# orottier/web-audio-api-rs

Measured on AMD Instinct MI355X. Metric: render quanta/sec (48kHz, 128-frame), higher is better.
Workload: dtype f64

## Files before the change

### web-audio-api-rs_amd/csrc/waa_internal.hpp

```cpp
#pragma once
#include <cstdint>
#include <cstdlib>

#include "waa_conv_noise.hpp"

namespace waa {

inline const char* measure_switch(const char* name) {
#ifdef WAA_MEASURE
  return getenv(name);
#else
  (void)name;
  return nullptr;
#endif
}

void raise_lds_limit(const void* kernel);

constexpr int RQ = 128;
constexpr int TILE_K = 32;
constexpr int TILE = 64 * TILE_K;
constexpr int QUANTA_PER_TILE = TILE / RQ;
constexpr int MAX_OPS = 12;
constexpr int MAX_INPUTS = 4;
constexpr int MAX_CH = 32;
constexpr int STATE_STRIDE = MAX_CH * 4;

struct ParamRef {
  const float* base;
  uint64_t stride;
  int32_t mode;
  int32_t pad;
};

struct SignalRef {
  float* base;
  uint64_t inst_stride;
  uint64_t ch_stride;
  int32_t nch;
  int32_t pad;
};

enum : uint32_t { Q_SILENT = 0, Q_FAST = 1, Q_SLOW = 2, Q_FAST_LOOP = 3 };
struct QRec {
  int64_t start;
  uint32_t mode;
  uint32_t pad;
};
struct SlowRec {
  int32_t prev;
  int32_t next;
  double k;
};
struct SrcSchedule {
  const QRec* qrec;
  const SlowRec* slow;
  const uint8_t* tile_fast;
};
struct SrcInst {
  const float* base;
// ... 304 lines not shown
  int32_t type;
  const uint32_t* wave_row;
  SignalRef out;
  uint64_t frames;
  uint32_t n_inst;
  uint32_t n_quanta;
  double sample_rate;
  const struct OscQuantum* table_q;
  const uint32_t* tq_row;
  const int64_t* active;
  const double* start_ratio;
  double* seg_phase;
  ParamRef post_gain[2];
  int32_t n_post;
  int32_t post_dup;
  const struct OscQuantum* fm_q;
  const uint32_t* fm_row;
  const float* fm_table;
  const uint32_t* fm_wave_row;
  int32_t fm_table_len, fm_type;
  ParamRef fm_gain;
  int32_t fm_has_gain;
  float fm_min, fm_max, fm_default;
  int32_t pa_on;
  float pa_min, pa_max, pa_default;
  ParamRef pa_intrinsic;
};
constexpr int OSC_SEGMENTS = 8;
struct OscQuantum {
  double phase;
  double incr;
  int16_t first, end;
  int32_t outside_nyquist;
};
void launch_osc(const OscDesc& d, void* stream);

constexpr int PERIODIC_WAVE_LEN = 8192;
struct PeriodicWaveDesc {
  const float* real;
  const float* imag;
  const uint32_t* normalize;
  const uint32_t* dst_row;
  float* tables;
  uint32_t n;
  uint32_t rows;
};
void launch_periodic_wave(const PeriodicWaveDesc& d, void* stream);

enum : int32_t { LI_NODE = 0, LI_DELAY_W = 1, LI_DELAY_R = 2 };
constexpr int LOOP_MAX_ITEMS = 24;
struct LoopItem {
  int32_t kind;
  int32_t nch_in;
  int32_t nch_out;
  int32_t interp;
  int32_t n_in;
  int32_t in_item[MAX_INPUTS];
  int32_t in_nch[MAX_INPUTS];
  SignalRef in_sig[MAX_INPUTS];
  SignalRef out;
  OpDesc op;
  int32_t writer_item;
  int32_t in_cycle;
  int32_t num_quanta;
  int32_t pad;
};
// ... 373 lines not shown
```

### web-audio-api-rs_amd/csrc/waa_kernels.hip

```cpp
#include <hip/hip_runtime.h>

#include <cstdlib>

#include "waa_curve.hpp"
#include "waa_internal.hpp"
#include "waa_mix.hpp"

namespace waa {

constexpr int LDS_ROW = TILE_K + 4;
constexpr int CARRY_BYTES = MAX_OPS * 8 * 4 * 8;

struct f4 {
  float x, y, z, w;
};

__device__ __forceinline__ float param_at(const ParamRef& p, uint32_t inst, uint32_t q, uint64_t frame) {
  if (p.mode == 0) return p.base[inst];
  if (p.mode == 1) return p.base[(uint64_t)inst * p.stride + q];
  return p.base[(uint64_t)inst * p.stride + frame];
}


template <int C, int K>
__device__ __forceinline__ void load_input(const InputRef& in, uint32_t inst, uint32_t tile, int lane, uint32_t n_quanta,
                                           float (&v)[C][K]) {
  constexpr int NV4 = K / 4;
  constexpr int TILE_FR = 64 * K;
  constexpr int QPT = K / 2;
  const uint64_t f_tile = (uint64_t)tile * TILE_FR;
  if (in.kind == IN_SIGNAL) {
#pragma unroll
    for (int c = 0; c < C; c++) {
      if (c < in.nch) {
        const float* p = in.sig.base + (uint64_t)inst * in.sig.inst_stride + (uint64_t)c * in.sig.ch_stride + f_tile;
#pragma unroll
        for (int j = 0; j < NV4; j++) {
          const bool inside = in.valid == 0 || f_tile + (uint64_t)(j * 256 + lane * 4) + 3 < in.valid;
// ... 191 lines not shown
__device__ __forceinline__ void gain_regs(float (&v)[C][K], int nch, const ParamRef& p0, uint32_t inst, uint32_t tile, int lane,
                                          uint32_t n_quanta) {
  constexpr int NV4 = K / 4;
  constexpr int TILE_FR = 64 * K;
  constexpr int QPT = K / 2;
#pragma unroll
  for (int j = 0; j < NV4; j++) {
    const uint32_t q = tile * QPT + j * 2 + (lane >> 5);
    const uint32_t qc = q < n_quanta ? q : n_quanta - 1;
    const uint64_t f = (uint64_t)tile * TILE_FR + j * 256 + lane * 4;
    if (p0.mode == 2) {
#pragma unroll
      for (int e = 0; e < 4; e++) {
        const uint64_t fc = f + e < (uint64_t)n_quanta * RQ ? f + e : (uint64_t)n_quanta * RQ - 1;
        const float g = p0.base[(uint64_t)inst * p0.stride + fc];
#pragma unroll
        for (int c = 0; c < C; c++)
          if (c < nch) v[c][j * 4 + e] *= g;
      }
    } else {
      const float g = param_at(p0, inst, qc, 0);
      const bool mute = fabsf(g) <= 1e-6f;
      const bool pass = fabsf(1.f - g) <= 1e-6f;
#pragma unroll
      for (int c = 0; c < C; c++)
        if (c < nch) {
#pragma unroll
          for (int e = 0; e < 4; e++) v[c][j * 4 + e] = mute ? 0.f : (pass ? v[c][j * 4 + e] : v[c][j * 4 + e] * g);
        }
    }
  }
}

struct Mat2 {
  double a, b, c, d;
};
__device__ __forceinline__ Mat2 matmul(const Mat2& x, const Mat2& y) {
  Mat2 r;
  r.a = __builtin_fma(x.a, y.a, x.b * y.c);
  r.b = __builtin_fma(x.a, y.b, x.b * y.d);
  r.c = __builtin_fma(x.c, y.a, x.d * y.c);
  r.d = __builtin_fma(x.c, y.b, x.d * y.d);
  return r;
}
__device__ __forceinline__ double shfl_up_d(double v, int delta) { return __shfl_up(v, delta, 64); }

template <int C>
__device__ __forceinline__ void biquad_op(const OpDesc& op, uint32_t inst, uint32_t tile, int lane, uint32_t n_quanta,
                                          float* lds, float (&v)[C][TILE_K], double* carry, const double* coef_inst) {
  constexpr int NV4 = TILE_K / 4;
  const int nch = op.nch_in;
#pragma unroll
  for (int c = 0; c < C; c++) {
    if (c < nch) {
      float* base = lds + c * (64 * LDS_ROW);
#pragma unroll
      for (int j = 0; j < NV4; j++) {
        const int row = j * 8 + (lane >> 3), col = (lane & 7) * 4;
        *reinterpret_cast<float4*>(base + row * LDS_ROW + col) =
            make_float4(v[c][j * 4 + 0], v[c][j * 4 + 1], v[c][j * 4 + 2], v[c][j * 4 + 3]);
      }
    }
  }
  __syncthreads();
  const bool per_frame = op.i0 == 2;
  const uint64_t f_lane = (uint64_t)tile * TILE + (uint64_t)lane * TILE_K;
// ... 121 lines not shown
            make_float4(yo[j * 4 + 0], yo[j * 4 + 1], yo[j * 4 + 2], yo[j * 4 + 3]);
    }
  }
  __syncthreads();
#pragma unroll
  for (int c = 0; c < C; c++) {
    if (c < nch) {
      const float* base = lds + c * (64 * LDS_ROW);
#pragma unroll
      for (int j = 0; j < NV4; j++) {
        const int row = j * 8 + (lane >> 3), col = (lane & 7) * 4;
        const float4 t = *reinterpret_cast<const float4*>(base + row * LDS_ROW + col);
        v[c][j * 4 + 0] = t.x;
        v[c][j * 4 + 1] = t.y;
        v[c][j * 4 + 2] = t.z;
        v[c][j * 4 + 3] = t.w;
      }
    }
  }
  __syncthreads();
}


__device__ __forceinline__ void stereo_gains_dev(float x, float& gl, float& gr) {
  const float PI_F = 3.14159265358979323846f;
  gl = sinf((1.f - x) * PI_F / 2.f);
  gr = sinf(x * PI_F / 2.f);
}

template <int C, int K, bool SERIAL, bool FANIN = true, bool PERSIST = false, bool NOSPILL = false>
__global__ __launch_bounds__(SERIAL ? 64 : 256)
    __attribute__((amdgpu_waves_per_eu((!SERIAL && FANIN && C == 2) ? (NOSPILL ? 5 : 6) : 1)))
void chain_kernel(const ChainDesc d) {
  extern __shared__ __attribute__((aligned(16))) float lds[];
  constexpr int NV4 = K / 4;
  constexpr int TILE_FR = 64 * K;
  constexpr int QPT = K / 2;
  const int lane = threadIdx.x & 63;
  const uint32_t n_tiles_k = (d.tile1 - d.tile0) * (TILE / TILE_FR);
  uint32_t inst, tile_first, tile_last;
  uint32_t tile_step = 1, per_block = 0;
  if (SERIAL) {
    inst = blockIdx.x;
    tile_first = d.tile0 * (TILE / TILE_FR);
    tile_last = d.tile1 * (TILE / TILE_FR);
  } else if (PERSIST) {
    inst = blockIdx.x;
    tile_first = d.tile0 * (TILE / TILE_FR) + (uint32_t)__builtin_amdgcn_readfirstlane((int)(threadIdx.x >> 6));
    tile_last = d.tile1 * (TILE / TILE_FR);
    tile_step = 4;
    per_block = d.persist_block / 4;
  } else {
    uint32_t blk = blockIdx.x;
    if (d.xcd_remap) {
      const uint32_t q = gridDim.x / 8, r = gridDim.x % 8, x = blk % 8, j = blk / 8;
      blk = x * q + (x < r ? x : r) + j;
    }
    const uint64_t wid = (uint64_t)blk * 4 + (uint32_t)__builtin_amdgcn_readfirstlane((int)(threadIdx.x >> 6));
    if (d.tile_major) {
      inst = (uint32_t)(wid % d.n_inst);
      tile_first = d.tile0 * (TILE / TILE_FR) + (uint32_t)(wid / d.n_inst);
      if (wid / d.n_inst >= n_tiles_k) inst = d.n_inst;
    } else {
      inst = (uint32_t)(wid / n_tiles_k);
      tile_first = d.tile0 * (TILE / TILE_FR) + (uint32_t)(wid % n_tiles_k);
    }
// ... 3 lines not shown
    if (d.lds_curve_op >= 0) {
      const int nn = d.ops[d.lds_curve_op].i0;
      const float* src = reinterpret_cast<const float*>(d.ops[d.lds_curve_op].ptr0);
      for (int i = threadIdx.x; i < nn; i += 256) lds[i] = src[i];
      __syncthreads();
    }
  }
  if (inst >= d.n_inst) return;
  __builtin_amdgcn_s_setreg(1 | (6 << 6) | (1 << 11), 0);

  double* carry_all = reinterpret_cast<double*>(lds + C * 64 * LDS_ROW);
  if constexpr (SERIAL) {
    for (int o = 0; o < d.n_ops; o++) {
      if (d.ops[o].kind == OP_BIQUAD) {
        const double* st = reinterpret_cast<const double*>(d.ops[o].ptr1) + (uint64_t)inst * STATE_STRIDE;
        if (lane < C * 4) carry_all[o * C * 4 + lane] = (lane >> 2) < d.ops[o].nch_in ? st[lane] : 0.;
      }
    }
    __syncthreads();
  }

  uint32_t done_in_block = 0;
  for (uint32_t tile = tile_first; tile < tile_last; tile += (PERSIST ? tile_step : 1u)) {
    if constexpr (PERSIST) {
      if (per_block) {
        if (done_in_block == per_block) {
          __syncthreads();
          done_in_block = 0;
        }
        done_in_block++;
      }
    }
    float v[C][K];
    if constexpr (!FANIN) {
      load_input<C, K>(d.in[0], inst, tile, lane, d.n_quanta, v);
      if (d.in[0].has_gain) gain_regs<C, K>(v, d.in[0].nch, d.in[0].gain, inst, tile, lane, d.n_quanta);
      mix_regs<C, K>(v, d.in[0].nch, d.in_nch, d.in_interp);
    } else {
#pragma unroll
      for (int c = 0; c < C; c++) {
#pragma unroll
        for (int i = 0; i < K; i++) v[c][i] = 0.f;
      }
#pragma nounroll
      for (int k = 0; k < d.n_inputs; k++) {
        float u[C][K];
        int lane_k = lane;
        asm volatile("" : "+v"(lane_k));
        load_input<C, K>(d.in[k], inst, tile, lane_k, d.n_quanta, u);
        if (d.in[k].has_gain) gain_regs<C, K>(u, d.in[k].nch, d.in[k].gain, inst, tile, lane_k, d.n_quanta);
        mix_regs<C, K>(u, d.in[k].nch, d.in_nch, d.in_interp);
#pragma unroll
        for (int c = 0; c < C; c++)
          if (c < d.in_nch) {
#pragma unroll
            for (int i = 0; i < K; i++) v[c][i] = k == 0 ? u[c][i] : v[c][i] + u[c][i];
          }
      }
    }
    for (int o = 0; o < d.n_ops; o++) {
      const OpDesc& op = d.ops[o];
      switch (op.kind) {
        case OP_GAIN:
          gain_regs<C, K>(v, op.nch_in, op.p0, inst, tile, lane, d.n_quanta);
          break;
        case OP_PARAM_ADD: {
          const float pmin = __int_as_float(op.i0), pmax = __int_as_float(op.i1), pdef = __int_as_float(op.i2);
#pragma unroll
          for (int j = 0; j < NV4; j++) {
            const uint32_t q = tile * QPT + j * 2 + (lane >> 5);
            const uint32_t qc = q < d.n_quanta ? q : d.n_quanta - 1;
            const uint64_t f = (uint64_t)tile * TILE_FR + j * 256 + lane * 4;
#pragma unroll
            for (int e = 0; e < 4; e++) {
              const uint64_t fc = f + e < (uint64_t)d.n_quanta * RQ ? f + e : (uint64_t)d.n_quanta * RQ - 1;
              float o1 = v[0][j * 4 + e] + param_at(op.p0, inst, qc, fc);
              o1 = o1 != o1 ? pdef : fminf(fmaxf(o1, pmin), pmax);
              v[0][j * 4 + e] = o1;
            }
          }
          break;
        }
        case OP_BIQUAD: {
          if constexpr (SERIAL) {
            const double* coef = reinterpret_cast<const double*>(op.ptr0) + (uint64_t)inst * op.u0;
            biquad_op<C>(op, inst, tile, lane, d.n_quanta, lds, v, carry_all + o * C * 4, coef);
          }
          break;
        }
        case OP_WAVESHAPER: {
          if (!SERIAL && o == d.lds_curve_op) {
#pragma unroll
            for (int c = 0; c < C; c++)
              if (c < op.nch_in) {
#pragma unroll
                for (int i = 0; i < K; i++)
                  v[c][i] = apply_curve_lds((const __attribute__((address_space(3))) float*)lds, op.i0, v[c][i]);
// ... 289 lines not shown
      return;
    }
    ChainDesc dd = d;
    dd.lds_curve_op = -1;
    dd.tile_major = 0;
    for (int k = 0; k < d.n_inputs; k++) dd.tile_major |= d.in[k].kind == IN_SOURCE;
    if (measure_switch("WAA_NO_TILE_MAJOR")) dd.tile_major = 0;
    dd.xcd_remap = !dd.tile_major && !measure_switch("WAA_NO_XCD_REMAP");
    for (int o = 0; o < d.n_ops; o++)
      if (d.ops[o].kind == OP_WAVESHAPER && d.ops[o].i0 > 0 && d.ops[o].i0 <= 8192) {
        dd.lds_curve_op = o;
        break;
      }
    const size_t lds = dd.lds_curve_op >= 0 ? (size_t)d.ops[dd.lds_curve_op].i0 * sizeof(float) : 0;
    const uint64_t waves = (uint64_t)d.n_inst * (d.tile1 - d.tile0) * (TILE / 256);
    dim3 grid((unsigned)((waves + 3) / 4)), block(256);
    if (d.persist_block) {
      grid = dim3(d.n_inst);
      dd.tile_major = 0;
      dd.xcd_remap = 0;
      if (d.n_inputs <= 1) {
        if (cmax <= 1)
          hipLaunchKernelGGL((chain_kernel<1, 4, false, false, true>), grid, block, lds, s, dd);
        else
          hipLaunchKernelGGL((chain_kernel<2, 4, false, false, true>), grid, block, lds, s, dd);
      } else if (cmax <= 1) {
        hipLaunchKernelGGL((chain_kernel<1, 4, false, true, true>), grid, block, lds, s, dd);
      } else {
        hipLaunchKernelGGL((chain_kernel<2, 4, false, true, true>), grid, block, lds, s, dd);
      }
      return;
    }
    if (d.n_inputs <= 1) {
      if (cmax <= 1)
        hipLaunchKernelGGL((chain_kernel<1, 4, false, false>), grid, block, lds, s, dd);
      else if (cmax <= 2)
        hipLaunchKernelGGL((chain_kernel<2, 4, false, false>), grid, block, lds, s, dd);
      else if (cmax <= 4)
        hipLaunchKernelGGL((chain_kernel<4, 4, false, false>), grid, block, lds, s, dd);
      else
        hipLaunchKernelGGL((chain_kernel<6, 4, false, false>), grid, block, lds, s, dd);
    } else if (cmax <= 1)
      hipLaunchKernelGGL((chain_kernel<1, 4, false>), grid, block, lds, s, dd);
    else if (cmax <= 2) {
      bool frame_pan = false;
      for (int o = 0; o < d.n_ops; o++)
        frame_pan |= (d.ops[o].kind == OP_STEREO_PAN || d.ops[o].kind == OP_PANNER) && d.ops[o].p0.mode == 2;
      if (frame_pan || measure_switch("WAA_CHAIN_NOSPILL"))
        hipLaunchKernelGGL((chain_kernel<2, 4, false, true, false, true>), grid, block, lds, s, dd);
      else
        hipLaunchKernelGGL((chain_kernel<2, 4, false>), grid, block, lds, s, dd);
    } else if (cmax <= 4)
      hipLaunchKernelGGL((chain_kernel<4, 4, false>), grid, block, lds, s, dd);
    else
      hipLaunchKernelGGL((chain_kernel<6, 4, false>), grid, block, lds, s, dd);
  }
}

}
```

### web-audio-api-rs_amd/csrc/waa_osc.hip

```cpp
#include <hip/hip_runtime.h>

#include "waa_internal.hpp"

namespace waa {

namespace {
__device__ __forceinline__ double unroll_phase(double phase) {
  if (phase >= 1.) return phase - 1.;
  if (phase < 0.) return phase + 1.;
  return phase;
}
__device__ __forceinline__ double unroll_phase_unbounded(double phase) {
  const double r = fmod(phase, 1.);
  return r < 0. ? r + 1. : r;
}
__device__ __forceinline__ double poly_blep(double t, double dt) {
  if (t < dt) {
    t /= dt;
    return t + t - t * t - 1.0;
  } else if (t > 1.0 - dt) {
    t = (t - 1.0) / dt;
    return __builtin_fma(t, t, t) + t + 1.0;
  }
  return 0.0;
}
__device__ __forceinline__ float table_sample(const float* table, int len, double phase) {
  const double position = phase * (double)len;
  const double floored = floor(position);
  const int prev_index = (int)floored >= len ? 0 : (int)floored;
  int next_index = prev_index + 1;
  if (next_index == len) next_index = 0;
  const float k = (float)(position - floored);
  return __builtin_fmaf(table[prev_index], 1.f - k, table[next_index] * k);
}
__device__ __forceinline__ float waveform_sample(int type, const float* table, int table_len, double phase, double phase_incr) {
  switch (type) {
    case 1: {
      double sample = phase < 0.5 ? 1.0 : -1.0;
      sample += poly_blep(phase, phase_incr);
      sample -= poly_blep(unroll_phase(phase + 0.5), phase_incr);
      return (float)sample;
    }
    case 2: {
      const double ph = unroll_phase(phase + 0.5);
      double sample = 2.0 * ph - 1.0;
      sample -= poly_blep(ph, phase_incr);
      return (float)sample;
    }
    case 3: {
      double sample = -4. * phase + 2.;
      if (sample > 1.)
        sample = 2. - sample;
      else if (sample < -1.)
        sample = -2. - sample;
      return (float)sample;
    }
    default: return table_sample(table, table_len, phase);
  }
}
__device__ __forceinline__ const float* table_of(const float* table, const uint32_t* wave_row, int table_len, uint32_t inst) {
  return wave_row ? table + (uint64_t)wave_row[inst] * (uint64_t)table_len : table;
}
}

namespace {
__device__ __forceinline__ void osc_store(const OscDesc& d, uint32_t inst, float* out, uint64_t f0, float (&r)[4]) {
#pragma unroll
  for (int k = 0; k < 2; k++)
    if (k < d.n_post) {
      const float g = d.post_gain[k].base[inst];
      const bool mute = fabsf(g) <= 1e-6f, pass = fabsf(1.f - g) <= 1e-6f;
#pragma unroll
      for (int e = 0; e < 4; e++) r[e] = mute ? 0.f : (pass ? r[e] : r[e] * g);
    }
  if (d.pa_on) {
    const uint32_t q = (uint32_t)(f0 / RQ), qc = q < d.n_quanta ? q : d.n_quanta - 1;
    const float iv = d.pa_intrinsic.mode == 0 ? d.pa_intrinsic.base[inst] : d.pa_intrinsic.base[(uint64_t)inst * d.pa_intrinsic.stride + qc];
#pragma unroll
    for (int e = 0; e < 4; e++) {
      const float o1 = r[e] + iv;
      r[e] = o1 != o1 ? d.pa_default : fminf(fmaxf(o1, d.pa_min), d.pa_max);
    }
  }
  *reinterpret_cast<float4*>(out + f0) = make_float4(r[0], r[1], r[2], r[3]);
  if (d.post_dup) *reinterpret_cast<float4*>(out + d.out.ch_stride + f0) = make_float4(r[0], r[1], r[2], r[3]);
}
}

__global__ __launch_bounds__(64) void osc_kernel(const OscDesc d) {
  const uint32_t inst = blockIdx.x * 64 + threadIdx.x;
  if (inst >= d.n_inst) return;
  __builtin_amdgcn_s_setreg(1 | (6 << 6) | (1 << 11), 0);
  float* out = d.out.base + (uint64_t)inst * d.out.inst_stride;
  const float* table = table_of(d.table, d.wave_row, d.table_len, inst);
  double start_time = d.start[inst];
  const double stop_time = d.stop[inst];
  const double sample_rate = d.sample_rate, dt = 1. / sample_rate, nyquist = sample_rate / 2.;
  double phase = 0.;
  bool started = false;
  const bool per_frame = d.frequency.mode == 2 || d.detune.mode == 2;
  for (uint32_t q = 0; q < d.n_quanta; q++) {
    const uint64_t f0 = (uint64_t)q * RQ;
    const double block_time = (double)f0 / sample_rate;
    const double next_block_time = block_time + dt * (double)RQ;
    float4* o4 = reinterpret_cast<float4*>(out + f0);
    if (stop_time <= block_time || start_time >= next_block_time) {
      for (int j = 0; j < RQ / 4; j++) o4[j] = make_float4(0.f, 0.f, 0.f, 0.f);
      continue;
    }
    double current_time = block_time;
    if (!started && start_time < current_time) start_time = current_time;
    auto generate = [&](bool outside_nyquist, double phase_incr) __attribute__((always_inline)) -> float {
      float v = 0.f;
      if (!(current_time < start_time || current_time >= stop_time)) {
        if (!started) {
          if (current_time > start_time) {
// ... 37 lines not shown
      for (int j = 0; j < RQ / 4; j++) {
        float r[4];
#pragma unroll
        for (int e = 0; e < 4; e++) {
          const uint64_t f = f0 + j * 4 + e;
          const float freq = d.frequency.mode == 0   ? d.frequency.base[inst]
                             : d.frequency.mode == 1 ? d.frequency.base[(uint64_t)inst * d.frequency.stride + q]
                                                     : d.frequency.base[(uint64_t)inst * d.frequency.stride + f];
          const float detune = d.detune.mode == 0   ? d.detune.base[inst]
                               : d.detune.mode == 1 ? d.detune.base[(uint64_t)inst * d.detune.stride + q]
                                                    : d.detune.base[(uint64_t)inst * d.detune.stride + f];
          const double computed_freq = (double)freq * exp2((double)detune / 1200.);
          const double phase_incr = computed_freq / sample_rate;
          r[e] = generate(fabs(computed_freq) >= nyquist, phase_incr);
        }
        o4[j] = make_float4(r[0], r[1], r[2], r[3]);
      }
    }
  }
  for (uint64_t f = (uint64_t)d.n_quanta * RQ; f < d.frames; f += 4) *reinterpret_cast<float4*>(out + f) = make_float4(0.f, 0.f, 0.f, 0.f);
}

__global__ __launch_bounds__(256) void osc_par_kernel(const OscDesc d) {
  const uint32_t inst = blockIdx.y;
  const uint64_t f0 = ((uint64_t)blockIdx.x * 256 + threadIdx.x) * 4;
  if (f0 >= d.frames) return;
  __builtin_amdgcn_s_setreg(1 | (6 << 6) | (1 << 11), 0);
  float* out = d.out.base + (uint64_t)inst * d.out.inst_stride;
  const float* table = table_of(d.table, d.wave_row, d.table_len, inst);
  const uint32_t q = (uint32_t)(f0 / RQ);
  float r[4] = {0.f, 0.f, 0.f, 0.f};
  if (q < d.n_quanta) {
    const OscQuantum oq = d.table_q[(uint64_t)d.tq_row[inst] * d.n_quanta + q];
    const int i0 = (int)(f0 % RQ);
#pragma unroll
    for (int e = 0; e < 4; e++) {
      const int i = i0 + e;
      if (i >= oq.first && i < oq.end && !oq.outside_nyquist) {
        const double x = __builtin_fma((double)(i - oq.first), oq.incr, oq.phase);
        double ph = x - floor(x);
        if (ph >= 1.) ph -= 1.;
        r[e] = waveform_sample(d.type, table, d.table_len, ph, oq.incr);
      }
    }
  }
  osc_store(d, inst, out, f0, r);
}

constexpr int OSC_LDS_SPAN = 8;
__global__ __launch_bounds__(256) void osc_par_lds_kernel(const OscDesc d) {
  __shared__ float lds_table[PERIODIC_WAVE_LEN];
  const uint32_t inst = blockIdx.y;
  __builtin_amdgcn_s_setreg(1 | (6 << 6) | (1 << 11), 0);
  const float4* src = reinterpret_cast<const float4*>(d.table + (uint64_t)d.wave_row[inst] * PERIODIC_WAVE_LEN);
#pragma unroll
  for (int k = 0; k < PERIODIC_WAVE_LEN / 4 / 256; k++) reinterpret_cast<float4*>(lds_table)[k * 256 + threadIdx.x] = src[k * 256 + threadIdx.x];
  __syncthreads();
  float* out = d.out.base + (uint64_t)inst * d.out.inst_stride;
  for (int s = 0; s < OSC_LDS_SPAN; s++) {
    const uint64_t f0 = (((uint64_t)blockIdx.x * OSC_LDS_SPAN + s) * 256 + threadIdx.x) * 4;
    if (f0 >= d.frames) break;
    const uint32_t q = (uint32_t)(f0 / RQ);
    float r[4] = {0.f, 0.f, 0.f, 0.f};
    if (q < d.n_quanta) {
      const OscQuantum oq = d.table_q[(uint64_t)d.tq_row[inst] * d.n_quanta + q];
      const int i0 = (int)(f0 % RQ);
#pragma unroll
      for (int e = 0; e < 4; e++) {
        const int i = i0 + e;
        if (i >= oq.first && i < oq.end && !oq.outside_nyquist) {
          const double x = __builtin_fma((double)(i - oq.first), oq.incr, oq.phase);
          double ph = x - floor(x);
          if (ph >= 1.) ph -= 1.;
          r[e] = table_sample(lds_table, PERIODIC_WAVE_LEN, ph);
        }
      }
    }
// ... 128 lines not shown
```

### web-audio-api-rs_amd/csrc/waa_plan.cpp

```cpp
#include <memory>

#include "waa_host.hpp"
#include "waa_plan_parts.hpp"

namespace waa {
namespace host {

int prepare_source_input(waa_batch* b, uint32_t id, InputRef* in);
int validate_plan(waa_batch* b);

int device_timeline_param(waa_batch* b, const ParamStore& p, ParamRef* ref) {
  if (p.dev_ready) {
    *ref = p.dev_ref;
    return 0;
  }
  std::vector<TlHeader> hdr(b->n_inst);
  std::vector<TlEvent> events;
  std::vector<float> curves;
  for (uint32_t i = 0; i < b->n_inst; i++) {
    TlHeader& h = hdr[i];
    std::memset(&h, 0, sizeof h);
    if (i < p.timelines.size() && p.timelines[i]) {
      p.timelines[i]->export_queue(&h, &events, &curves);
    } else {
// ... 1256 lines not shown
  if (int e = refuse_nested_source_modulation(b)) return e;
  if (int e = static_channel_counts(b, pass)) return e;
  ph.reset();
  ph.reset(new PlanTrace("phase: silence / count replay"));
  if (int e = replay_channel_counts(b, pass)) return e;
  ph.reset();
  ph.reset(new PlanTrace("phase: folds + materialisation + views"));
  choose_frozen_sources(b, pass);
  choose_block_loops(b, pass);
  choose_folded_delays(b, pass);
  choose_materialisation(b, pass);
  fold_fan_in_edges(b, pass);
  choose_source_views(b, pass);
  fold_biquad_into_convolver(b, pass);
  ph.reset();
  ph.reset(new PlanTrace("phase: units + steps"));
  order_units(b, pass);
  b->steps.clear();
  if (b->prepass && pass.dynamic(b))
    return fail(WAA_ERR_OUT_OF_SCOPE, "the graph that modulates a source's playbackRate / detune needs exact per-quantum channel counts: out of scope");
  if (pass.dynamic(b)) {
    if (int e = refuse_static_only_nodes(b, pass, false)) return e;
    return plan_dynamic_groups(b, pass);
  }
  for (const Unit& unit : pass.units) {
    bool restart = false;
    if (int e = unit.scc >= 0 ? plan_loop_unit(b, pass, unit.scc, &restart) : plan_single(b, pass, unit.id)) return e;
    if (restart) return restart_plan(b);
  }
  fuse_echo_tails(b);
  ring_feed_forward_echoes(b);
  fuse_fm_operators(b);
  fuse_lfo_params(b);
  ph.reset();
  ph.reset(new PlanTrace("phase: validate"));
  if (measure_switch("WAA_DEBUG_REVERSE_PLAN")) std::reverse(b->steps.begin(), b->steps.end());
  if (int e = validate_plan(b)) return e;
  b->planned = true;
  return 0;
}

}
}
```

### web-audio-api-rs_amd/csrc/waa_plan_check.cpp

```cpp
#include <array>
#include <set>

#include "waa_host.hpp"
#include "waa_plan_parts.hpp"

namespace waa {
namespace host {

void io_param(const ParamRef& p, StepIo& io) {
  if (p.base && p.mode == 2) io.reads.push_back(p.base);
}
void io_input(const InputRef& in, StepIo& io) {
  if (in.kind == IN_SIGNAL || (in.kind == IN_DELAYED && !in.feedback)) io.reads.push_back(in.sig.base);
  if (in.kind == IN_CONSTANT) io_param(in.offset, io);
  if (in.has_gain) io_param(in.gain, io);
}
static StepIo step_io_raw(const Step& st);
StepIo step_io(const waa_batch* b, const Step& st) {
  StepIo io = step_io_raw(st);
  if (!b->view_owner.empty())
    for (const void*& r : io.reads) {
      auto it = b->view_owner.find(r);
      if (it != b->view_owner.end()) r = it->second;
    }
  return io;
}
static StepIo step_io_raw(const Step& st) {
  StepIo io;
  switch (st.kind) {
    case StepKind::Chain: {
      const ChainDesc& c = st.chain;
      for (int k = 0; k < c.n_inputs; k++) io_input(c.in[k], io);
      for (int o = 0; o < c.n_ops; o++) {
        const OpDesc& op = c.ops[o];
        io_param(op.p0, io);
        io_param(op.p1, io);
        io_param(op.p2, io);
        io_param(op.p3, io);
        io_param(op.p4, io);
        if (op.kind == OP_BIQUAD && op.i0 == 2) io.reads.push_back(op.ptr0);
      }
      io.writes.push_back(c.out.base);
      break;
// ... 119 lines not shown
```

### web-audio-api-rs_amd/csrc/waa_plan_parts.hpp

```cpp
#pragma once
#include <map>
#include <set>
#include <vector>

#include "waa_host.hpp"

namespace waa {
namespace host {

struct StepIo {
  std::vector<const void*> reads, writes;
  bool feedback_reader = false;
};
struct OrderCtx;
struct Unit {
  int scc;
  uint32_t id;
};
struct PlanPass {
  std::vector<uint32_t> items;
  std::vector<uint8_t> muted;
  std::vector<int> scc_of;
  int n_scc = 0;
  bool mixed_buffer_counts = false;
// ... 45 lines not shown
int flush_group(DynPlan& p);
int plan_dyn_convolver(DynPlan& p, uint32_t id);
int plan_quantum_blocked_loop(DynPlan& p, const std::vector<uint32_t>& verts);
constexpr uint32_t VTX_READER = 0x80000000u;

int device_timeline_param(waa_batch* b, const ParamStore& p, ParamRef* ref);
int upload_param(waa_batch* b, const ParamStore& p, ParamRef* ref);
int param_mode(const Node& n, size_t k);
int node_param(waa_batch* b, uint32_t id, size_t k, ParamRef* ref);
int build_edge_input(waa_batch* b, uint32_t head, int ie, InputRef* out);
int upload_values(waa_batch* b, const std::vector<float>& host, int mode, ParamRef* ref);
int computed_in_nch(const Node& n, int maxc);
bool order_visit(OrderCtx& c, uint32_t v);
void plan_note(waa_batch* b, const char* fmt, ...);
const char* input_kind_name(int k);
const char* op_name(int k);
int slot_for(waa_batch* b, const char* name);
int push_chain_step(waa_batch* b, const std::vector<InputRef>& inputs, int in_nch, int in_interp, const std::vector<OpDesc>& ops, const SignalRef& out);
int temp_signal(waa_batch* b, int nch, SignalRef* out);
int emit_segments(waa_batch* b, std::vector<InputRef> inputs, int in_nch, int in_interp, const std::vector<OpDesc>& ops, const SignalRef& out);
bool is_delay(const waa_batch* b, uint32_t id);
void vertex_targets(const waa_batch* b, uint32_t v, const std::vector<uint8_t>& cut, std::vector<uint32_t>& out);
int materialise_automation(waa_batch* b);
int source_code_rows(waa_batch* b, uint32_t id, uint64_t cs, std::vector<uint8_t>* out);
int build_plan(waa_batch* b);
void io_param(const ParamRef& p, StepIo& io);
void io_input(const InputRef& in, StepIo& io);
StepIo step_io(const waa_batch* b, const Step& st);
int validate_plan(waa_batch* b);
void fuse_echo_tails(waa_batch* b);
void ring_feed_forward_echoes(waa_batch* b);
void fuse_fm_operators(waa_batch* b);
void fuse_lfo_params(waa_batch* b);
int plan_delay_writer(waa_batch* b, uint32_t id);
int plan_folded_delay_line(waa_batch* b, uint32_t id);
int plan_delay_reader(waa_batch* b, uint32_t id);
uint32_t loop_block_tiles(waa_batch* b, const std::vector<uint32_t>& loop_items);
int plan_loop(waa_batch* b, const std::vector<uint32_t>& loop_items);
int prepare_source_input(waa_batch* b, uint32_t id, InputRef* in);
int widen_narrow_buffers(waa_batch* b, Node& n, uint32_t nch);
int reduce_fan_in(waa_batch* b, std::vector<InputRef>& ins, int in_nch, int interp);
int premix_ordered_inputs(waa_batch* b, uint32_t id, std::vector<InputRef>& ins);
int node_input_signal(waa_batch* b, uint32_t id, SignalRef* out_sig, const SignalRef* target = nullptr, uint64_t* valid = nullptr);
int plan_oscillator(waa_batch* b, uint32_t id);
int conv_block_size(const waa_batch* b, const Node& n);
bool conv_fold_biquad_into_ir(const waa_batch* b, Node& conv, const Node& q);
int plan_convolver(waa_batch* b, uint32_t id);
int plan_compressor(waa_batch* b, uint32_t id);
int plan_shaper_per_instance(waa_batch* b, uint32_t id);
int desugar_output_ports(waa_batch* b);
int plan_splitter(waa_batch* b, uint32_t id, bool producer_in_loop);
int plan_splitter_port(waa_batch* b, uint32_t id);
int plan_merger(waa_batch* b, uint32_t id);
int emit_node_ops(waa_batch* b, uint32_t id, int cur_nch, bool head, std::vector<OpDesc>& ops, int* out_nch);
void default_channel_config(Node& n, uint32_t n_out);

}
}
```

### web-audio-api-rs_amd/csrc/waa_plan_sources.cpp

```cpp
#include <array>
#include <set>

#include "waa_host.hpp"
#include "waa_plan_parts.hpp"

namespace waa {
namespace host {

int widen_narrow_buffers(waa_batch* b, Node& n, uint32_t nch) {
  std::map<const float*, DeviceBuffer> done;
  for (auto& bf : n.bufs) {
    if (!bf.valid || bf.nch >= nch) continue;
    auto it = done.find(bf.base);
    if (it == done.end()) {
      const uint64_t stride = std::max<uint64_t>(bf.ch_stride, 4);
      float* d = nullptr;
      int e = dev_alloc(b, &d, (size_t)nch * stride, true);
      if (e) return e;
      const size_t all = (size_t)nch * stride * sizeof(float), plane = (size_t)bf.frames * sizeof(float);
      if (b->dry) {
        std::memset(d, 0, all);
        for (uint32_t c = 0; c < bf.nch && plane; c++) std::memcpy(d + (size_t)c * stride, bf.base + (size_t)c * bf.ch_stride, plane);
      } else {
        HIP_TRY(hipMemsetAsync(d, 0, all, b->stream));
// ... 613 lines not shown
    int mi = -1;
    for (size_t k = 0; k < pi; k++) {
      const Step& st = b->steps[k];
      if (st.kind == StepKind::Osc && st.group < 0 && !st.echo_fused && st.osc.table_q && !st.osc.pa_on && st.osc.out.base == ch.in[0].sig.base) mi = (int)k;
    }
    if (mi < 0) continue;
    Step& ms = b->steps[(size_t)mi];
    if (ms.osc.post_dup || ms.osc.out.nch != 1 || ms.osc.n_post + (ch.in[0].has_gain ? 1 : 0) > 2 ||
        ms.osc.out.inst_stride != ch.in[0].sig.inst_stride || ch.out.inst_stride != ms.osc.out.inst_stride)
      continue;
    bool shared = false;
    for (size_t k = 0; k < b->steps.size() && !shared; k++) {
      if (k == pi) continue;
      const StepIo io = step_io(b, b->steps[k]);
      for (const void* r : io.reads) shared |= r == (const void*)ms.osc.out.base;
    }
    for (const Node& an : b->nodes)
      if (an.live && (an.desc.kind == WAA_NODE_ANALYSER || an.desc.kind == WAA_NODE_DESTINATION) && an.sig.base == ms.osc.out.base) shared = true;
    if (shared) continue;
    OscDesc& d = ms.osc;
    if (ch.in[0].has_gain) d.post_gain[d.n_post++] = ch.in[0].gain;
    d.pa_on = 1;
    d.pa_intrinsic = ch.ops[0].p0;
    std::memcpy(&d.pa_min, &ch.ops[0].i0, 4);
    std::memcpy(&d.pa_max, &ch.ops[0].i1, 4);
    std::memcpy(&d.pa_default, &ch.ops[0].i2, 4);
    d.out = ch.out;
    ps.echo_fused = true;
    plan_note(b, "LFO: launch %zu (the param's sum: %sintrinsic value, clamp) is folded into the store of the oscillator that drives it (launch %d)", pi,
              ch.in[0].has_gain ? "depth gain, " : "", mi);
  }
}

}
}
```

Measured before the change: 2.916 billion.

## Inline LFO oscillator evaluation into its single gain-consumer chain kernel

Adds a planner pass that finds an oscillator step whose per-frame param buffer has exactly one reader, a simple non-serial chain using it as a gain. That oscillator launch is dropped and the chain kernel evaluates the waveform, post-gains and the param clamp in registers from a device-side LfoParam record. This removes one kernel launch plus a full write and read of the per-frame param table. In exchange the chain kernel does more arithmetic and carries more register state in a new template variant. Shared waveform helpers move into a common header.

```diff
diff --git a/web-audio-api-rs_amd/csrc/waa_internal.hpp b/web-audio-api-rs_amd/csrc/waa_internal.hpp
--- a/web-audio-api-rs_amd/csrc/waa_internal.hpp
+++ b/web-audio-api-rs_amd/csrc/waa_internal.hpp
@@ -26,6 +26,7 @@
 constexpr int MAX_CH = 32;
 constexpr int STATE_STRIDE = MAX_CH * 4;
 
+constexpr int32_t PARAM_GENERATED = 4;
 struct ParamRef {
   const float* base;
   uint64_t stride;
@@ -396,6 +397,18 @@
   double incr;
   int16_t first, end;
   int32_t outside_nyquist;
+};
+struct LfoParam {
+  const OscQuantum* table_q;
+  const uint32_t* tq_row;
+  const float* table;
+  int32_t table_len, type;
+  ParamRef post_gain[2];
+  int32_t n_post;
+  uint32_t n_quanta;
+  ParamRef pa_intrinsic;
+  float pa_min, pa_max, pa_default;
+  int32_t pad;
 };
 void launch_osc(const OscDesc& d, void* stream);
 
diff --git a/web-audio-api-rs_amd/csrc/waa_kernels.hip b/web-audio-api-rs_amd/csrc/waa_kernels.hip
--- a/web-audio-api-rs_amd/csrc/waa_kernels.hip
+++ b/web-audio-api-rs_amd/csrc/waa_kernels.hip
@@ -4,6 +4,7 @@
 
 #include "waa_curve.hpp"
 #include "waa_internal.hpp"
+#include "waa_lfo.hpp"
 #include "waa_mix.hpp"
 
 namespace waa {
@@ -261,6 +262,21 @@
   }
 }
 
+template <int C, int K>
+__device__ __forceinline__ void generated_gain_regs(float (&v)[C][K], int nch, const LfoValue4 (&begun)[K / 4]) {
+#pragma unroll
+  for (int j = 0; j < K / 4; j++) {
+    float g[4];
+    lfo_value4_finish(begun[j], g);
+#pragma unroll
+    for (int e = 0; e < 4; e++) {
+#pragma unroll
+      for (int c = 0; c < C; c++)
+        if (c < nch) v[c][j * 4 + e] *= g[e];
+    }
+  }
+}
+
 struct Mat2 {
   double a, b, c, d;
 };
@@ -448,6 +464,7 @@
 __global__ __launch_bounds__(SERIAL ? 64 : 256)
     __attribute__((amdgpu_waves_per_eu((!SERIAL && FANIN && C == 2) ? (NOSPILL ? 5 : 6) : 1)))
 void chain_kernel(const ChainDesc d) {
+  constexpr bool LFOGEN = !SERIAL && !FANIN && !PERSIST && NOSPILL;
   extern __shared__ __attribute__((aligned(16))) float lds[];
   constexpr int NV4 = K / 4;
   constexpr int TILE_FR = 64 * K;
@@ -517,9 +534,21 @@
       }
     }
     float v[C][K];
+    LfoValue4 begun[NV4];
+    if constexpr (LFOGEN) {
+      const float* rec = d.in[0].has_gain && d.in[0].gain.mode == PARAM_GENERATED ? d.in[0].gain.base : nullptr;
+      for (int o = 0; o < d.n_ops && !rec; o++)
+        if (d.ops[o].kind == OP_GAIN && d.ops[o].p0.mode == PARAM_GENERATED) rec = d.ops[o].p0.base;
+#pragma unroll
+      for (int j = 0; j < NV4; j++)
+        begun[j] = lfo_value4_begin(reinterpret_cast<const LfoParam*>(rec), inst, (uint64_t)tile * TILE_FR + j * 256, lane);
+    }
     if constexpr (!FANIN) {
       load_input<C, K>(d.in[0], inst, tile, lane, d.n_quanta, v);
-      if (d.in[0].has_gain) gain_regs<C, K>(v, d.in[0].nch, d.in[0].gain, inst, tile, lane, d.n_quanta);
+      if (LFOGEN && d.in[0].has_gain && d.in[0].gain.mode == PARAM_GENERATED)
+        generated_gain_regs<C, K>(v, d.in[0].nch, begun);
+      else if (d.in[0].has_gain)
+        gain_regs<C, K>(v, d.in[0].nch, d.in[0].gain, inst, tile, lane, d.n_quanta);
       mix_regs<C, K>(v, d.in[0].nch, d.in_nch, d.in_interp);
     } else {
 #pragma unroll
@@ -547,7 +576,10 @@
       const OpDesc& op = d.ops[o];
       switch (op.kind) {
         case OP_GAIN:
-          gain_regs<C, K>(v, op.nch_in, op.p0, inst, tile, lane, d.n_quanta);
+          if (LFOGEN && op.p0.mode == PARAM_GENERATED)
+            generated_gain_regs<C, K>(v, op.nch_in, begun);
+          else
+            gain_regs<C, K>(v, op.nch_in, op.p0, inst, tile, lane, d.n_quanta);
           break;
         case OP_PARAM_ADD: {
           const float pmin = __int_as_float(op.i0), pmax = __int_as_float(op.i1), pdef = __int_as_float(op.i2);
@@ -903,6 +935,15 @@
       return;
     }
     if (d.n_inputs <= 1) {
+      bool generated = d.n_inputs == 1 && d.in[0].has_gain && d.in[0].gain.mode == PARAM_GENERATED;
+      for (int o = 0; o < d.n_ops; o++) generated |= d.ops[o].kind == OP_GAIN && d.ops[o].p0.mode == PARAM_GENERATED;
+      if (generated && cmax <= 2) {
+        if (cmax <= 1)
+          hipLaunchKernelGGL((chain_kernel<1, 4, false, false, false, true>), grid, block, lds, s, dd);
+        else
+          hipLaunchKernelGGL((chain_kernel<2, 4, false, false, false, true>), grid, block, lds, s, dd);
+        return;
+      }
       if (cmax <= 1)
         hipLaunchKernelGGL((chain_kernel<1, 4, false, false>), grid, block, lds, s, dd);
       else if (cmax <= 2)
diff --git a/web-audio-api-rs_amd/csrc/waa_lfo.hpp b/web-audio-api-rs_amd/csrc/waa_lfo.hpp
--- /dev/null
+++ b/web-audio-api-rs_amd/csrc/waa_lfo.hpp
@@ -0,0 +1,217 @@
+#pragma once
+#include <hip/hip_runtime.h>
+
+#include <type_traits>
+
+#include "waa_internal.hpp"
+
+namespace waa {
+
+__device__ __forceinline__ OscQuantum load_global(const OscQuantum* p) {
+  OscQuantum r;
+  r.phase = load_global(&p->phase);
+  r.incr = load_global(&p->incr);
+  r.first = load_global(&p->first);
+  r.end = load_global(&p->end);
+  r.outside_nyquist = load_global(&p->outside_nyquist);
+  return r;
+}
+
+#define WAA_CONST_AS __attribute__((address_space(4)))
+template <class T>
+__device__ __forceinline__ T load_uniform(const T* p) {
+  static_assert(sizeof(T) <= 8, "scalar types only");
+  return *(const WAA_CONST_AS T*)p;
+}
+__device__ __forceinline__ OscQuantum load_uniform(const OscQuantum* p) {
+  OscQuantum r;
+  r.phase = load_uniform(&p->phase);
+  r.incr = load_uniform(&p->incr);
+  r.first = load_uniform(&p->first);
+  r.end = load_uniform(&p->end);
+  r.outside_nyquist = load_uniform(&p->outside_nyquist);
+  return r;
+}
+
+__device__ __forceinline__ double unroll_phase(double phase) {
+  if (phase >= 1.) return phase - 1.;
+  if (phase < 0.) return phase + 1.;
+  return phase;
+}
+__device__ __forceinline__ double poly_blep(double t, double dt) {
+  if (t < dt) {
+    t /= dt;
+    return t + t - t * t - 1.0;
+  } else if (t > 1.0 - dt) {
+    t = (t - 1.0) / dt;
+    return __builtin_fma(t, t, t) + t + 1.0;
+  }
+  return 0.0;
+}
+struct TableTap {
+  int prev_index, next_index;
+  float k;
+};
+__device__ __forceinline__ TableTap table_tap(int len, double phase) {
+  const double position = phase * (double)len;
+  const double floored = floor(position);
+  TableTap t;
+  t.prev_index = (int)floored >= len ? 0 : (int)floored;
+  t.next_index = t.prev_index + 1;
+  if (t.next_index == len) t.next_index = 0;
+  t.k = (float)(position - floored);
+  return t;
+}
+__device__ __forceinline__ float table_mix(float prev, float next, float k) { return __builtin_fmaf(prev, 1.f - k, next * k); }
+template <bool GLOBAL = false>
+__device__ __forceinline__ float table_sample(const float* table, int len, double phase) {
+  const TableTap t = table_tap(len, phase);
+  const float prev = GLOBAL ? load_global(table + t.prev_index) : table[t.prev_index];
+  const float next = GLOBAL ? load_global(table + t.next_index) : table[t.next_index];
+  return table_mix(prev, next, t.k);
+}
+__device__ __forceinline__ float waveform_sample(int type, const float* table, int table_len, double phase, double phase_incr) {
+  switch (type) {
+    case 1: {
+      double sample = phase < 0.5 ? 1.0 : -1.0;
+      sample += poly_blep(phase, phase_incr);
+      sample -= poly_blep(unroll_phase(phase + 0.5), phase_incr);
+      return (float)sample;
+    }
+    case 2: {
+      const double ph = unroll_phase(phase + 0.5);
+      double sample = 2.0 * ph - 1.0;
+      sample -= poly_blep(ph, phase_incr);
+      return (float)sample;
+    }
+    case 3: {
+      double sample = -4. * phase + 2.;
+      if (sample > 1.)
+        sample = 2. - sample;
+      else if (sample < -1.)
+        sample = -2. - sample;
+      return (float)sample;
+    }
+    default: return table_sample<true>(table, table_len, phase);
+  }
+}
+
+struct LfoWave4 {
+  float prev[4], next[4], k[4];
+  bool on[4];
+  bool from_table;
+};
+__device__ __forceinline__ LfoWave4 lfo_wave4_begin(int type, const float* table, int table_len, const OscQuantum& oq, int i0, int step) {
+  LfoWave4 w;
+  double ph[4];
+#pragma unroll
+  for (int e = 0; e < 4; e++) {
+    const int i = i0 + e * step;
+    w.on[e] = i >= oq.first && i < oq.end && !oq.outside_nyquist;
+    const double x = __builtin_fma((double)(i - oq.first), oq.incr, oq.phase);
+    double p = x - floor(x);
+    if (p >= 1.) p -= 1.;
+    ph[e] = w.on[e] ? p : 0.;
+    w.prev[e] = w.next[e] = w.k[e] = 0.f;
+  }
+  w.from_table = false;
+  auto computed = [&](auto type_c) __attribute__((always_inline)) {
+#pragma unroll
+    for (int e = 0; e < 4; e++)
+      if (w.on[e]) w.prev[e] = waveform_sample(decltype(type_c)::value, table, table_len, ph[e], oq.incr);
+  };
+  switch (type) {
+    case 1: computed(std::integral_constant<int, 1>{}); return w;
+    case 2: computed(std::integral_constant<int, 2>{}); return w;
+    case 3: computed(std::integral_constant<int, 3>{}); return w;
+    default: break;
+  }
+  w.from_table = true;
+#pragma unroll
+  for (int e = 0; e < 4; e++) {
+    const TableTap t = table_tap(table_len, ph[e]);
+    w.k[e] = t.k;
+    w.prev[e] = load_global(table + t.prev_index);
+    w.next[e] = load_global(table + t.next_index);
+  }
+  return w;
+}
+__device__ __forceinline__ void lfo_wave4_finish(const LfoWave4& w, float (&r)[4]) {
+#pragma unroll
+  for (int e = 0; e < 4; e++) r[e] = !w.from_table ? w.prev[e] : w.on[e] ? table_mix(w.prev[e], w.next[e], w.k[e]) : 0.f;
+}
+__device__ __forceinline__ void lfo_wave4(int type, const float* table, int table_len, const OscQuantum& oq, int i0, int step, float (&r)[4]) {
+  const LfoWave4 w = lfo_wave4_begin(type, table, table_len, oq, i0, step);
+  lfo_wave4_finish(w, r);
+}
+
+__device__ __forceinline__ void lfo_post4(const float (&gain)[2], int n_post, bool pa_on, float iv, float pa_min, float pa_max, float pa_default,
+                                          float (&r)[4]) {
+#pragma unroll
+  for (int k = 0; k < 2; k++)
+    if (k < n_post) {
+      const float g = gain[k];
+      const bool mute = fabsf(g) <= 1e-6f, pass = fabsf(1.f - g) <= 1e-6f;
+#pragma unroll
+      for (int e = 0; e < 4; e++) r[e] = mute ? 0.f : (pass ? r[e] : r[e] * g);
+    }
+  if (pa_on) {
+#pragma unroll
+    for (int e = 0; e < 4; e++) {
+      const float o1 = r[e] + iv;
+      r[e] = o1 != o1 ? pa_default : fminf(fmaxf(o1, pa_min), pa_max);
+    }
+  }
+}
+
+struct LfoValue4 {
+  LfoWave4 w;
+  float gain[2], iv, pa_min, pa_max, pa_default;
+  int n_post;
+};
+__device__ __forceinline__ LfoValue4 lfo_value4_begin(const LfoParam* rec, uint32_t inst, uint64_t f_wave, int lane) {
+  const OscQuantum* table_q = load_uniform(&rec->table_q);
+  const uint32_t* tq_row = load_uniform(&rec->tq_row);
+  const float* table = load_uniform(&rec->table);
+  const int table_len = load_uniform(&rec->table_len), type = load_uniform(&rec->type), n_post = load_uniform(&rec->n_post);
+  const uint32_t n_quanta = load_uniform(&rec->n_quanta);
+  const float pa_min = load_uniform(&rec->pa_min), pa_max = load_uniform(&rec->pa_max), pa_default = load_uniform(&rec->pa_default);
+  const float* iv_base = load_uniform(&rec->pa_intrinsic.base);
+  const uint64_t iv_stride = load_uniform(&rec->pa_intrinsic.stride);
+  const int iv_mode = load_uniform(&rec->pa_intrinsic.mode);
+  float gain[2] = {0.f, 0.f};
+#pragma unroll
+  for (int k = 0; k < 2; k++)
+    if (k < n_post) gain[k] = load_uniform(load_uniform(&rec->post_gain[k].base) + inst);
+
+  const uint32_t q_lo = (uint32_t)(f_wave / RQ);
+  const uint32_t qa = q_lo < n_quanta ? q_lo : n_quanta - 1, qb = q_lo + 1 < n_quanta ? q_lo + 1 : n_quanta - 1;
+  const OscQuantum* row = table_q + (uint64_t)load_uniform(tq_row + inst) * n_quanta;
+  const OscQuantum a = load_uniform(row + qa), b = load_uniform(row + qb);
+  const bool hi = lane >= 32;
+  OscQuantum oq;
+  oq.phase = hi ? b.phase : a.phase;
+  oq.incr = hi ? b.incr : a.incr;
+  oq.first = hi ? b.first : a.first;
+  oq.end = hi ? b.end : a.end;
+  oq.outside_nyquist = hi ? b.outside_nyquist : a.outside_nyquist;
+  const float iv_a = load_uniform(iv_base + (iv_mode == 0 ? (uint64_t)inst : (uint64_t)inst * iv_stride + qa));
+  const float iv_b = load_uniform(iv_base + (iv_mode == 0 ? (uint64_t)inst : (uint64_t)inst * iv_stride + qb));
+  const bool live = q_lo + (hi ? 1u : 0u) < n_quanta;
+  LfoValue4 v;
+  v.w = lfo_wave4_begin(type, table, table_len, oq, live ? (lane & 31) * 4 : RQ - 1, live ? 1 : 0);
+  v.gain[0] = gain[0];
+  v.gain[1] = gain[1];
+  v.iv = hi ? iv_b : iv_a;
+  v.pa_min = pa_min;
+  v.pa_max = pa_max;
+  v.pa_default = pa_default;
+  v.n_post = n_post;
+  return v;
+}
+__device__ __forceinline__ void lfo_value4_finish(const LfoValue4& v, float (&r)[4]) {
+  lfo_wave4_finish(v.w, r);
+  lfo_post4(v.gain, v.n_post, true, v.iv, v.pa_min, v.pa_max, v.pa_default, r);
+}
+
+}
diff --git a/web-audio-api-rs_amd/csrc/waa_osc.hip b/web-audio-api-rs_amd/csrc/waa_osc.hip
--- a/web-audio-api-rs_amd/csrc/waa_osc.hip
+++ b/web-audio-api-rs_amd/csrc/waa_osc.hip
@@ -1,87 +1,28 @@
 #include <hip/hip_runtime.h>
 
 #include "waa_internal.hpp"
+#include "waa_lfo.hpp"
 
 namespace waa {
 
 namespace {
-__device__ __forceinline__ double unroll_phase(double phase) {
-  if (phase >= 1.) return phase - 1.;
-  if (phase < 0.) return phase + 1.;
-  return phase;
-}
 __device__ __forceinline__ double unroll_phase_unbounded(double phase) {
   const double r = fmod(phase, 1.);
   return r < 0. ? r + 1. : r;
 }
-__device__ __forceinline__ double poly_blep(double t, double dt) {
-  if (t < dt) {
-    t /= dt;
-    return t + t - t * t - 1.0;
-  } else if (t > 1.0 - dt) {
-    t = (t - 1.0) / dt;
-    return __builtin_fma(t, t, t) + t + 1.0;
-  }
-  return 0.0;
-}
-__device__ __forceinline__ float table_sample(const float* table, int len, double phase) {
-  const double position = phase * (double)len;
-  const double floored = floor(position);
-  const int prev_index = (int)floored >= len ? 0 : (int)floored;
-  int next_index = prev_index + 1;
-  if (next_index == len) next_index = 0;
-  const float k = (float)(position - floored);
-  return __builtin_fmaf(table[prev_index], 1.f - k, table[next_index] * k);
-}
-__device__ __forceinline__ float waveform_sample(int type, const float* table, int table_len, double phase, double phase_incr) {
-  switch (type) {
-    case 1: {
-      double sample = phase < 0.5 ? 1.0 : -1.0;
-      sample += poly_blep(phase, phase_incr);
-      sample -= poly_blep(unroll_phase(phase + 0.5), phase_incr);
-      return (float)sample;
-    }
-    case 2: {
-      const double ph = unroll_phase(phase + 0.5);
-      double sample = 2.0 * ph - 1.0;
-      sample -= poly_blep(ph, phase_incr);
-      return (float)sample;
-    }
-    case 3: {
-      double sample = -4. * phase + 2.;
-      if (sample > 1.)
-        sample = 2. - sample;
-      else if (sample < -1.)
-        sample = -2. - sample;
-      return (float)sample;
-    }
-    default: return table_sample(table, table_len, phase);
-  }
-}
 __device__ __forceinline__ const float* table_of(const float* table, const uint32_t* wave_row, int table_len, uint32_t inst) {
   return wave_row ? table + (uint64_t)wave_row[inst] * (uint64_t)table_len : table;
 }
-}
-
-namespace {
 __device__ __forceinline__ void osc_store(const OscDesc& d, uint32_t inst, float* out, uint64_t f0, float (&r)[4]) {
+  float gain[2] = {0.f, 0.f}, iv = 0.f;
 #pragma unroll
   for (int k = 0; k < 2; k++)
-    if (k < d.n_post) {
-      const float g = d.post_gain[k].base[inst];
-      const bool mute = fabsf(g) <= 1e-6f, pass = fabsf(1.f - g) <= 1e-6f;
-#pragma unroll
-      for (int e = 0; e < 4; e++) r[e] = mute ? 0.f : (pass ? r[e] : r[e] * g);
-    }
+    if (k < d.n_post) gain[k] = d.post_gain[k].base[inst];
   if (d.pa_on) {
     const uint32_t q = (uint32_t)(f0 / RQ), qc = q < d.n_quanta ? q : d.n_quanta - 1;
-    const float iv = d.pa_intrinsic.mode == 0 ? d.pa_intrinsic.base[inst] : d.pa_intrinsic.base[(uint64_t)inst * d.pa_intrinsic.stride + qc];
-#pragma unroll
-    for (int e = 0; e < 4; e++) {
-      const float o1 = r[e] + iv;
-      r[e] = o1 != o1 ? d.pa_default : fminf(fmaxf(o1, d.pa_min), d.pa_max);
-    }
-  }
+    iv = d.pa_intrinsic.mode == 0 ? d.pa_intrinsic.base[inst] : d.pa_intrinsic.base[(uint64_t)inst * d.pa_intrinsic.stride + qc];
+  }
+  lfo_post4(gain, d.n_post, d.pa_on != 0, iv, d.pa_min, d.pa_max, d.pa_default, r);
   *reinterpret_cast<float4*>(out + f0) = make_float4(r[0], r[1], r[2], r[3]);
   if (d.post_dup) *reinterpret_cast<float4*>(out + d.out.ch_stride + f0) = make_float4(r[0], r[1], r[2], r[3]);
 }
@@ -185,17 +126,7 @@
   float r[4] = {0.f, 0.f, 0.f, 0.f};
   if (q < d.n_quanta) {
     const OscQuantum oq = d.table_q[(uint64_t)d.tq_row[inst] * d.n_quanta + q];
-    const int i0 = (int)(f0 % RQ);
-#pragma unroll
-    for (int e = 0; e < 4; e++) {
-      const int i = i0 + e;
-      if (i >= oq.first && i < oq.end && !oq.outside_nyquist) {
-        const double x = __builtin_fma((double)(i - oq.first), oq.incr, oq.phase);
-        double ph = x - floor(x);
-        if (ph >= 1.) ph -= 1.;
-        r[e] = waveform_sample(d.type, table, d.table_len, ph, oq.incr);
-      }
-    }
+    lfo_wave4(d.type, table, d.table_len, oq, (int)(f0 % RQ), 1, r);
   }
   osc_store(d, inst, out, f0, r);
 }
diff --git a/web-audio-api-rs_amd/csrc/waa_plan.cpp b/web-audio-api-rs_amd/csrc/waa_plan.cpp
--- a/web-audio-api-rs_amd/csrc/waa_plan.cpp
+++ b/web-audio-api-rs_amd/csrc/waa_plan.cpp
@@ -1312,6 +1312,7 @@
   ring_feed_forward_echoes(b);
   fuse_fm_operators(b);
   fuse_lfo_params(b);
+  if (int e = inline_lfo_params(b)) return e;
   ph.reset();
   ph.reset(new PlanTrace("phase: validate"));
   if (measure_switch("WAA_DEBUG_REVERSE_PLAN")) std::reverse(b->steps.begin(), b->steps.end());
diff --git a/web-audio-api-rs_amd/csrc/waa_plan_check.cpp b/web-audio-api-rs_amd/csrc/waa_plan_check.cpp
--- a/web-audio-api-rs_amd/csrc/waa_plan_check.cpp
+++ b/web-audio-api-rs_amd/csrc/waa_plan_check.cpp
@@ -9,6 +9,7 @@
 
 void io_param(const ParamRef& p, StepIo& io) {
   if (p.base && p.mode == 2) io.reads.push_back(p.base);
+  if (p.base && p.mode == PARAM_GENERATED) io.reads.push_back(p.base);
 }
 void io_input(const InputRef& in, StepIo& io) {
   if (in.kind == IN_SIGNAL || (in.kind == IN_DELAYED && !in.feedback)) io.reads.push_back(in.sig.base);
diff --git a/web-audio-api-rs_amd/csrc/waa_plan_parts.hpp b/web-audio-api-rs_amd/csrc/waa_plan_parts.hpp
--- a/web-audio-api-rs_amd/csrc/waa_plan_parts.hpp
+++ b/web-audio-api-rs_amd/csrc/waa_plan_parts.hpp
@@ -101,6 +101,7 @@
 void ring_feed_forward_echoes(waa_batch* b);
 void fuse_fm_operators(waa_batch* b);
 void fuse_lfo_params(waa_batch* b);
+int inline_lfo_params(waa_batch* b);
 int plan_delay_writer(waa_batch* b, uint32_t id);
 int plan_folded_delay_line(waa_batch* b, uint32_t id);
 int plan_delay_reader(waa_batch* b, uint32_t id);
diff --git a/web-audio-api-rs_amd/csrc/waa_plan_sources.cpp b/web-audio-api-rs_amd/csrc/waa_plan_sources.cpp
--- a/web-audio-api-rs_amd/csrc/waa_plan_sources.cpp
+++ b/web-audio-api-rs_amd/csrc/waa_plan_sources.cpp
@@ -669,5 +669,84 @@
   }
 }
 
-}
-}
+int inline_lfo_params(waa_batch* b) {
+  if (measure_switch("WAA_NO_LFO_FOLD") || measure_switch("WAA_NO_LFO_INLINE")) return 0;
+  for (size_t mi = 0; mi < b->steps.size(); mi++) {
+    Step& ms = b->steps[mi];
+    const OscDesc& od = ms.osc;
+    if (ms.kind != StepKind::Osc || ms.group >= 0 || ms.qgroup >= 0 || ms.echo_fused || !od.pa_on || !od.table_q || od.wave_row ||
+        od.post_dup || od.out.nch != 1 || od.pa_intrinsic.mode > 1 || od.n_quanta != b->n_quanta)
+      continue;
+    const void* table = od.out.base;
+    int ri = -1, readers = 0;
+    for (size_t k = 0; k < b->steps.size(); k++) {
+      if (k == mi) continue;
+      const StepIo io = step_io(b, b->steps[k]);
+      bool reads = false;
+      for (const void* r : io.reads) reads |= r == table;
+      if (reads) {
+        readers++;
+        ri = (int)k;
+      }
+    }
+    for (const Node& an : b->nodes)
+      if (an.live && (an.desc.kind == WAA_NODE_ANALYSER || an.desc.kind == WAA_NODE_DESTINATION) && (const void*)an.sig.base == table) readers = 2;
+    if (readers != 1 || ri < (int)mi) continue;
+    Step& rs = b->steps[(size_t)ri];
+    if (rs.kind != StepKind::Chain || rs.group >= 0 || rs.qgroup >= 0 || rs.prologue || rs.echo_fused || rs.echo_ff || rs.echo_fb >= 0 ||
+        rs.chain.n_inputs != 1 || rs.chain.in[0].kind != IN_SOURCE || rs.cmax > 2)
+      continue;
+    ChainDesc& ch = rs.chain;
+    bool serial = false;
+    for (int o = 0; o < ch.n_ops; o++) serial |= ch.ops[o].kind == OP_BIQUAD;
+    if (serial) continue;
+    ParamRef* slot = nullptr;
+    int uses = 0;
+    bool taken = false;
+    auto use = [&](ParamRef& p, bool gain) {
+      taken |= p.mode == PARAM_GENERATED;
+      if (p.mode != 2 || (const void*)p.base != table) return;
+      uses++;
+      if (gain && p.stride == od.out.inst_stride) slot = &p;
+    };
+    for (int k = 0; k < ch.n_inputs; k++) {
+      use(ch.in[k].offset, false);
+      if (ch.in[k].has_gain) use(ch.in[k].gain, true);
+    }
+    for (int o = 0; o < ch.n_ops; o++) {
+      OpDesc& op = ch.ops[o];
+      use(op.p0, op.kind == OP_GAIN);
+      use(op.p1, false);
+      use(op.p2, false);
+      use(op.p3, false);
+      use(op.p4, false);
+    }
+    if (uses != 1 || !slot || taken) continue;
+    LfoParam rec{};
+    rec.table_q = od.table_q;
+    rec.tq_row = od.tq_row;
+    rec.table = od.table;
+    rec.table_len = od.table_len;
+    rec.type = od.type;
+    rec.post_gain[0] = od.post_gain[0];
+    rec.post_gain[1] = od.post_gain[1];
+    rec.n_post = od.n_post;
+    rec.n_quanta = od.n_quanta;
+    rec.pa_intrinsic = od.pa_intrinsic;
+    rec.pa_min = od.pa_min;
+    rec.pa_max = od.pa_max;
+    rec.pa_default = od.pa_default;
+    LfoParam* d_rec = nullptr;
+    if (int e = dev_upload(b, &d_rec, std::vector<LfoParam>(1, rec))) return e;
+    slot->base = reinterpret_cast<const float*>(d_rec);
+    slot->stride = 0;
+    slot->mode = PARAM_GENERATED;
+    ms.echo_fused = true;
+    plan_note(b, "LFO: launch %zu (the oscillator that writes the param's per-frame table) is not run: launch %d, the table's only reader, evaluates it per frame in registers",
+              mi, ri);
+  }
+  return 0;
+}
+
+}
+}
```

New measurement: 2.725 billion. 6.5% lower.
